# Justin900429/autonomous_driving_with_diffusion_model

Measured on AMD Instinct MI355X. Metric: denoising-steps/sec, higher is better.
Workload: dtype f32

## Files before the change

### autonomous_driving_with_diffusion_model_amd/csrc/conv2d_hs.hip

```cpp
#include <type_traits>
#include <stdlib.h>

#include "adx_common.h"
#include "conv2d_internal.h"
#include "conv2d_hs_common.h"

namespace adx {

template <bool AFFINE = true>
__device__ __forceinline__ void cells_store32(float (&v)[16], const float* sc, const float* sh, int cl0, const float (*res8)[8],
                                              bool relu, __amdgpu_buffer_rsrc_t yrsrc, uint32_t vcell, uint32_t so, uint32_t cplane,
                                              float& amax) {
  float lm = 0.f;
#pragma unroll
  for (int i = 0; i < 2; ++i)
#pragma unroll
    for (int j = 0; j < 4; ++j) {
      const auto sw = __builtin_amdgcn_permlane32_swap(f2u(v[8 * i + j]), f2u(v[8 * i + 4 + j]), false, false);
      v[8 * i + j] = u2f(sw[0]);
      v[8 * i + 4 + j] = u2f(sw[1]);
    }
#pragma unroll
  for (int i = 0; i < 2; ++i) {
    float o[8];
// ... 755 lines not shown
      const u32x4* wa0 = wl + (i & 1) * WST + wa_lane;
      load_w(s + 2 < nstages ? s + 2 : nstages - 1, i & 1);
      if ((i + 1) % 3 < PIT) load_p(s + 4 < nstages ? (s + 4) / 3 : nchunks - 1, (i + 1) % 3, i & 1);
      __builtin_amdgcn_sched_barrier(0);
#pragma unroll
      for (int kw = 0; kw < K; ++kw) {
        f16x8 A[2][2], B[2][2];
#pragma unroll
        for (int pl = 0; pl < 2; ++pl) {
#pragma unroll
          for (int m = 0; m < 2; ++m) A[pl][m] = __builtin_bit_cast(f16x8, wa0[(kw * 2 + pl) * 128 + m * 32]);
#pragma unroll
          for (int r = 0; r < 2; ++r) B[pl][r] = __builtin_bit_cast(f16x8, pb0[pl * PLANE + (r + kh) * PW + kw]);
        }
#pragma unroll
        for (int r = 0; r < 2; ++r)
#pragma unroll
          for (int m = 0; m < 2; ++m) {
            accm[r][m] = hs_mfma(A[0][m], B[0][r], accm[r][m]);
            accl[r][m] = hs_mfma(A[0][m], B[1][r], accl[r][m]);
            accl[r][m] = hs_mfma(A[1][m], B[0][r], accl[r][m]);
          }
        if (kw == 0) {
          store_w((i + 1) & 1, (i + 1) & 1);
          if (i % 3 < PIT) store_p((i + 1) & 1, i % 3, ((i + 3) / 3) & 1);
        }
      }
      __syncthreads();
    }
  }

  HS_TRACE(3);
  const int ox = VROW ? xl : ox0 + ecol;
  const uint32_t plane_ob = (uint32_t)(a.OH * a.OW) * (uint32_t)sizeof(float);
  const size_t img = (size_t)n * a.Cout * a.OH * a.OW;
  const int img_bytes = (int)(uint32_t)((VROW ? (uint32_t)a.N : 1u) * (uint32_t)a.Cout * plane_ob);
  const uint32_t img_off = VROW ? (uint32_t)nl * (uint32_t)a.Cout * plane_ob : 0u;
  float* const ybase = a.ksplit > 1 ? a.part + (size_t)kpart * a.part_stride : a.y;
  const __amdgpu_buffer_rsrc_t yrsrc = __builtin_amdgcn_make_buffer_rsrc(ybase + img, 0, img_bytes, 0x00020000);
  const __amdgpu_buffer_rsrc_t rrsrc = __builtin_amdgcn_make_buffer_rsrc(
      const_cast<float*>(a.res != nullptr ? a.res + img : a.y), 0, a.res != nullptr ? img_bytes : 0, 0x00020000);
  const float* sst = ss + slab * 64;
  const uint32_t cbase_o = (uint32_t)cout0 * plane_ob;
  const uint32_t cplane = (uint32_t)(a.OH * a.OW) * 16u;
  const uint32_t cell0 = (uint32_t)(cout0 >> 3) * 2u * cplane;
  bool inside[2];
  uint32_t pix[2];
#pragma unroll
  for (int rr = 0; rr < 2; ++rr) {
    const int oy = oy0 + rowpair * 2 + rr;
    inside[rr] = lane_valid && oy < a.OH && ox < a.OW;
    pix[rr] = (uint32_t)(oy * a.OW + ox);
  }
  float amax = 0.f;
  if constexpr (YCELLS) {
    const uint32_t khoff = (uint32_t)khalf * 2u * cplane;
    uint32_t vcell[2], vres[2];
#pragma unroll
    for (int rr = 0; rr < 2; ++rr) {
      vcell[rr] = inside[rr] ? img_off + pix[rr] * 16u + khoff : kOutside;
      vres[rr] = !inside[rr] ? kOutside : a.res_cells ? vcell[rr] : img_off + pix[rr] * 4u + (uint32_t)(8 * khalf) * plane_ob;
    }
    uint32_t rraw[2][2][2][8];
#pragma unroll
    for (int rr = 0; rr < 2; ++rr)
#pragma unroll
      for (int half = 0; half < 2; ++half)
#pragma unroll
        for (int i = 0; i < 2; ++i) {
          if (a.res_cells) {
            const uint32_t so = cell0 + (uint32_t)(half * 4 + 2 * i) * 2u * cplane;
            const u32x4 h4 = __builtin_amdgcn_raw_buffer_load_b128(rrsrc, vres[rr], so, 0);
            const u32x4 l4 = __builtin_amdgcn_raw_buffer_load_b128(rrsrc, vres[rr], so + cplane, 0);
#pragma unroll
            for (int j = 0; j < 4; ++j) { rraw[rr][half][i][j] = h4[j]; rraw[rr][half][i][4 + j] = l4[j]; }
          } else {
#pragma unroll
            for (int j = 0; j < 8; ++j)
              rraw[rr][half][i][j] = __builtin_amdgcn_raw_buffer_load_b32(rrsrc, vres[rr], cbase_o + (uint32_t)(half * 32 + 16 * i + j) * plane_ob, 0);
          }
        }
#ifdef ADX_HS_TRACE
    asm volatile("s_waitcnt vmcnt(0)" ::: "memory");
    HS_TRACE(6);
#endif
#pragma unroll
    for (int rr = 0; rr < 2; ++rr)
#pragma unroll
      for (int half = 0; half < 2; ++half) {
        float v[16];
#pragma unroll
        for (int r = 0; r < 16; ++r) v[r] = accm[rr][half][r] + accl[rr][half][r] * (1.f / kLoScale);
        float res8[2][8];
#pragma unroll
        for (int i = 0; i < 2; ++i) {
          if (a.res_cells) {
            half4(rraw[rr][half][i][0], rraw[rr][half][i][1], rraw[rr][half][i][4], rraw[rr][half][i][5], res8[i]);
            half4(rraw[rr][half][i][2], rraw[rr][half][i][3], rraw[rr][half][i][6], rraw[rr][half][i][7], res8[i] + 4);
          } else {
#pragma unroll
            for (int j = 0; j < 8; ++j) res8[i][j] = u2f(rraw[rr][half][i][j]);
          }
        }
        cells_store32(v, sst, sst + 64 * CT, half * 32 + 8 * khalf, res8, a.relu != 0, yrsrc, vcell[rr],
                      cell0 + (uint32_t)(half * 4) * 2u * cplane, cplane, amax);
      }
  } else {
  uint32_t voff[2];
#pragma unroll
  for (int rr = 0; rr < 2; ++rr) voff[rr] = inside[rr] ? img_off + pix[rr] * 4u + (uint32_t)(4 * khalf) * plane_ob : kOutside;
  float rv[2][2][16];
  if constexpr (STATS != 2) {
#pragma unroll
  for (int rr = 0; rr < 2; ++rr)
#pragma unroll
    for (int half = 0; half < 2; ++half)
#pragma unroll
      for (int r = 0; r < 16; ++r) {
        const int cu = half * 32 + (r & 3) + 8 * (r >> 2);
        rv[rr][half][r] = __builtin_bit_cast(float, __builtin_amdgcn_raw_buffer_load_b32(rrsrc, voff[rr], cbase_o + cu * plane_ob, 0));
      }
  }
#ifdef ADX_HS_TRACE
  asm volatile("s_waitcnt vmcnt(0)" ::: "memory");
  HS_TRACE(6);
#endif
  if constexpr (STATS != 0) {
    float* red = reinterpret_cast<float*>(smem_raw);
    const bool val0 = voff[0] != kOutside, val1 = voff[1] != kOutside;
    auto park = [&](int half, int r, float sm, float sq) {
      sm += hs_dpp<0xB1>(sm);  sq += hs_dpp<0xB1>(sq);
      sm += hs_dpp<0x4E>(sm);  sq += hs_dpp<0x4E>(sq);
      sm += hs_dpp<0x141>(sm); sq += hs_dpp<0x141>(sq);
      sm += hs_dpp<0x140>(sm); sq += hs_dpp<0x140>(sq);
      if ((lane & 15) == 0) {
        float* d = red + (((wave * 4 + (lane >> 4)) * 32) + half * 16 + r) * 2;
        d[0] = sm;
        d[1] = sq;
      }
    };
    if constexpr (STATS == 1) {
#pragma unroll
      for (int half = 0; half < 2; ++half)
#pragma unroll
        for (int r = 0; r < 16; ++r) {
          const float v0 = val0 ? (accm[0][half][r] + accl[0][half][r] * (1.f / kLoScale)) * xs_inv : 0.f;
          const float v1 = val1 ? (accm[1][half][r] + accl[1][half][r] * (1.f / kLoScale)) * xs_inv : 0.f;
          park(half, r, v0 + v1, v0 * v0 + v1 * v1);
        }
    } else {
#pragma unroll
      for (int rr = 0; rr < 2; ++rr)
#pragma unroll
        for (int half = 0; half < 2; ++half)
#pragma unroll
          for (int r = 0; r < 16; ++r) accm[rr][half][r] = (accm[rr][half][r] + accl[rr][half][r] * (1.f / kLoScale)) * xs_inv;
      const __amdgpu_buffer_rsrc_t wrsrc = __builtin_amdgcn_make_buffer_rsrc(const_cast<float*>(a.bs_raw + img), 0, img_bytes, 0x00020000);
      const bool mask_bits = a.bs_mask == 1 && a.bs_bits != nullptr;
      const bool mask_out = a.bs_mask == 1 && !mask_bits;
      const __amdgpu_buffer_rsrc_t orsrc = __builtin_amdgcn_make_buffer_rsrc(
          const_cast<float*>(mask_out ? a.bs_out + img : a.y), 0, mask_out ? img_bytes : 0, 0x00020000);
      const uint32_t bplane = (uint32_t)(a.OH * a.OW);
      const __amdgpu_buffer_rsrc_t brsrc = __builtin_amdgcn_make_buffer_rsrc(
          const_cast<uint8_t*>(mask_bits ? a.bs_bits + (size_t)n * (a.Cout >> 3) * bplane : reinterpret_cast<const uint8_t*>(a.y)), 0,
          mask_bits ? (int)((VROW ? (uint32_t)a.N : 1u) * (uint32_t)(a.Cout >> 3) * bplane) : 0, 0x00020000);
      uint32_t boff[2];
#pragma unroll
      for (int rr = 0; rr < 2; ++rr)
        boff[rr] = inside[rr] ? (VROW ? (uint32_t)nl * (uint32_t)(a.Cout >> 3) * bplane : 0u) + pix[rr] : kOutside;
      const bool res_masked = a.res_bits != nullptr;
      const __amdgpu_buffer_rsrc_t qrsrc = __builtin_amdgcn_make_buffer_rsrc(
          const_cast<uint8_t*>(res_masked ? a.res_bits + (size_t)n * (a.Cout >> 3) * bplane : reinterpret_cast<const uint8_t*>(a.y)), 0,
          res_masked ? (int)((VROW ? (uint32_t)a.N : 1u) * (uint32_t)(a.Cout >> 3) * bplane) : 0, 0x00020000);
      const float* bsw = bsl + slab * 64;
      const uint32_t use_bit = mask_bits ? 1u : 0u, use_out = mask_out ? 1u : 0u, use_raw = 1u - use_bit - use_out;
      const uint32_t v0u = val0 ? 1u : 0u, v1u = val1 ? 1u : 0u;
      float dmx = 0.f;
#pragma unroll
      for (int half = 0; half < 2; ++half) {
        float rs_[2][16], rw_[2][16], ro_[2][16];
#pragma unroll
        for (int rr = 0; rr < 2; ++rr)
#pragma unroll
          for (int r = 0; r < 16; ++r) {
            const uint32_t so = cbase_o + (uint32_t)(half * 32 + (r & 3) + 8 * (r >> 2)) * plane_ob;
            rs_[rr][r] = __builtin_bit_cast(float, __builtin_amdgcn_raw_buffer_load_b32(rrsrc, voff[rr], so, 0));
            rw_[rr][r] = __builtin_bit_cast(float, __builtin_amdgcn_raw_buffer_load_b32(wrsrc, voff[rr], so, 0));
            ro_[rr][r] = 0.f;
          }
        if (mask_out) {
#pragma unroll
          for (int rr = 0; rr < 2; ++rr)
#pragma unroll
            for (int r = 0; r < 16; ++r) {
              const uint32_t so = cbase_o + (uint32_t)(half * 32 + (r & 3) + 8 * (r >> 2)) * plane_ob;
              ro_[rr][r] = __builtin_bit_cast(float, __builtin_amdgcn_raw_buffer_load_b32(orsrc, voff[rr], so, 0));
            }
        }
        if (res_masked) {
#pragma unroll
          for (int rr = 0; rr < 2; ++rr)
#pragma unroll
            for (int q = 0; q < 4; ++q) {
              const uint32_t m = (uint32_t)__builtin_amdgcn_raw_buffer_load_b8(qrsrc, boff[rr], ((uint32_t)(cout0 >> 3) + (uint32_t)(half * 4 + q)) * bplane, 0)
                                 >> (4 * khalf);
#pragma unroll
              for (int i = 0; i < 4; ++i)
                if (!((m >> i) & 1u)) rs_[rr][4 * q + i] = 0.f;
            }
        }
        uint32_t mb[2][4] = {{0u, 0u, 0u, 0u}, {0u, 0u, 0u, 0u}};
        if (mask_bits) {
#pragma unroll
          for (int rr = 0; rr < 2; ++rr)
#pragma unroll
            for (int q = 0; q < 4; ++q)
              mb[rr][q] = (uint32_t)__builtin_amdgcn_raw_buffer_load_b8(brsrc, boff[rr], ((uint32_t)(cout0 >> 3) + (uint32_t)(half * 4 + q)) * bplane, 0)
                          >> (4 * khalf);
        }
#pragma unroll
        for (int r = 0; r < 16; ++r) {
          const int cu = half * 32 + (r & 3) + 8 * (r >> 2);
          const int cl = cu + 4 * khalf;
          const float mu = bsw[cl], rsd = bsw[64 * CT + cl], msc = bsw[2 * 64 * CT + cl], msh = bsw[3 * 64 * CT + cl];
          float p[2], q[2];
#pragma unroll
          for (int rr = 0; rr < 2; ++rr) {
            const float y = accm[rr][half][r] + rs_[rr][r];
            __builtin_amdgcn_raw_buffer_store_b32(__builtin_bit_cast(uint32_t, y), yrsrc, voff[rr], cbase_o + cu * plane_ob, 0);
            const uint32_t on_bit = (mb[rr][r >> 2] >> (r & 3)) & 1u, on_out = ro_[rr][r] > 0.f ? 1u : 0u;
            const uint32_t on_raw = __builtin_fmaf(rw_[rr][r], msc, msh) > 0.f ? 1u : 0u;
            const bool keep = ((rr == 0 ? v0u : v1u) & ((on_bit & use_bit) | (on_out & use_out) | (on_raw & use_raw))) != 0u;
            p[rr] = keep ? y : 0.f;
            q[rr] = p[rr] * ((rw_[rr][r] - mu) * rsd);
            dmx = __builtin_fmaxf(dmx, __builtin_fabsf(p[rr]));
          }
          park(half, r, p[0] + p[1], q[0] + q[1]);
        }
      }
#pragma unroll
      for (int off = 32; off > 0; off >>= 1) dmx = __builtin_fmaxf(dmx, __shfl_xor(dmx, off, 64));
      if (lane == 0) red[4096 + wave] = dmx;
    }
    __syncthreads();
    if (STATS == 2 && tid >= 2 * 64 * CT && tid < 2 * 64 * CT + CT) {
      const int sl = tid - 2 * 64 * CT;
      constexpr int WPS = (NT / 64) / CT;
      float t = 0.f;
#pragma unroll
      for (int w = 0; w < WPS; ++w) t = __builtin_fmaxf(t, red[4096 + (MODE == 2 ? sl * WPS + w : w)]);
      const int p = (n * a.tiles_y + ty) * a.tiles_x + tx;
      a.stats_part[(size_t)a.Cout * 2 * a.stats_p + (size_t)(ct * CT + sl) * a.stats_p + p] = t;
    }
    if (tid < 2 * 64 * CT) {
      const int which = tid & 1, chs = tid >> 1, sl = chs >> 6, ch = chs & 63;
      const int c5 = ch & 31, kh2 = (c5 >> 2) & 1, r = (c5 & 3) + 4 * (c5 >> 3), idx32 = (ch >> 5) * 16 + r;
      constexpr int WPS = (NT / 64) / CT;
      float t = 0.f;
#pragma unroll
      for (int w = 0; w < WPS; ++w)
#pragma unroll
        for (int j = 0; j < 2; ++j) t += red[((((MODE == 2 ? sl * WPS + w : w) * 4 + kh2 * 2 + j) * 32) + idx32) * 2 + which];
      const int p = (n * a.tiles_y + ty) * a.tiles_x + tx;
      a.stats_part[((size_t)((ct * CT + sl) * kHsCout + ch) * 2 + which) * a.stats_p + p] = t;
    }
  }
  auto finish = [&](auto relu) {
#pragma unroll
    for (int rr = 0; rr < 2; ++rr) {
      float lm = 0.f;
#pragma unroll
      for (int half = 0; half < 2; ++half)
#pragma unroll
        for (int r = 0; r < 16; ++r) {
          const int cu = half * 32 + (r & 3) + 8 * (r >> 2);
          const int cl = cu + 4 * khalf;
          float v = (accm[rr][half][r] + accl[rr][half][r] * (1.f / kLoScale)) * xs_inv;
          v = v * sst[cl] + sst[64 * CT + cl];
          v += rv[rr][half][r];
          if (decltype(relu)::value) v = __builtin_fmaxf(v, 0.f);
          lm = fp16_amax(lm, v);
          __builtin_amdgcn_raw_buffer_store_b32(__builtin_bit_cast(uint32_t, v), yrsrc, voff[rr], cbase_o + cu * plane_ob, 0);
        }
      amax = fp16_amax(amax, inside[rr] ? lm : 0.f);
    }
  };
  if constexpr (STATS != 2) {
    if (a.relu) finish(std::true_type{}); else finish(std::false_type{});
  }
  }
  range_flag(a.status, out_of_fp16(amax));
  HS_TRACE(4);
#ifdef ADX_HS_TRACE
  __builtin_amdgcn_s_waitcnt(0);
  asm volatile("s_waitcnt vmcnt(0)" ::: "memory");
  HS_TRACE(5);
#endif
}

constexpr int kStemSteps = 11;
constexpr int kStemPP = 72;
constexpr int kStemPH = 21;

struct StemFrags { f16x8 A[2][2], B[2]; };
__device__ __forceinline__ void stem_tile(const u32x4* wa0, const uint32_t* pb0, int khalf, f32x16 (&accm)[2], f32x16 (&accl)[2]) {
  constexpr int CP = kStemPH * kStemPP, PLANEH = 3 * CP;
#pragma unroll
  for (int m = 0; m < 2; ++m)
#pragma unroll
    for (int i = 0; i < 16; ++i) { accm[m][i] = 0.f; accl[m][i] = 0.f; }
  auto fetch = [&](StemFrags& f, int step) {
    const int c0 = 2 * step, c1 = 2 * step + 1 > 20 ? 20 : 2 * step + 1;
    const int off0 = ((c0 / 7) * CP + (c0 % 7) * kStemPP) / 2, off1 = ((c1 / 7) * CP + (c1 % 7) * kStemPP) / 2;
    const uint32_t* pb = pb0 + (khalf ? off1 : off0);
#pragma unroll
    for (int pl = 0; pl < 2; ++pl) {
#pragma unroll
      for (int m = 0; m < 2; ++m) f.A[pl][m] = __builtin_bit_cast(f16x8, wa0[(step * 2 + pl) * 128 + m * 32]);
      const uint32_t* q = pb + pl * (PLANEH / 2);
      u32x4 v;
      v[0] = q[0]; v[1] = q[1]; v[2] = q[2]; v[3] = q[3];
      f.B[pl] = __builtin_bit_cast(f16x8, v);
    }
  };
  StemFrags fr[2];
  fetch(fr[0], 0);
#pragma unroll
  for (int step = 0; step < kStemSteps; ++step) {
    if (step + 1 < kStemSteps) fetch(fr[(step + 1) & 1], step + 1);
    __builtin_amdgcn_sched_barrier(0);
    const StemFrags& f = fr[step & 1];
#pragma unroll
    for (int m = 0; m < 2; ++m) {
      accm[m] = hs_mfma(f.A[0][m], f.B[0], accm[m]);
      accl[m] = hs_mfma(f.A[0][m], f.B[1], accl[m]);
      accl[m] = hs_mfma(f.A[1][m], f.B[0], accl[m]);
    }
    __builtin_amdgcn_sched_barrier(0);
  }
}

constexpr int kStemStageItems = 3 * kStemPH / 7;
template <bool U8>
struct StemStager {
  float pv[kStemStageItems][2];
  float amax = 0.f;
  __device__ __forceinline__ void load(const Conv2dArgs& a, __amdgpu_buffer_rsrc_t xrsrc, int r0, int ix, int iy0) {
    constexpr uint32_t kOutside = 0xC0000000u;
    const bool act = r0 < 7;
    const bool ok0 = act && ix >= 0 && ix < a.W, ok1 = act && ix + 1 >= 0 && ix + 1 < a.W;
    const size_t hw = (size_t)a.H * a.W;
#pragma unroll
    for (int k = 0; k < kStemStageItems; ++k) {
      const int rc = r0 + 7 * k;
      const int c = (rc >= kStemPH) + (rc >= 2 * kStemPH), iy = iy0 + rc - kStemPH * c;
      const bool rok = iy >= 0 && iy < a.H;
      const bool v0 = rok && ok0, v1 = rok && ok1;
      if (U8) {
#pragma clang fp contract(off)
        const uint32_t brow = (uint32_t)(iy * a.W) * 3u + (uint32_t)c;
        const uint32_t b0 = __builtin_amdgcn_raw_buffer_load_b8(xrsrc, v0 ? brow + (uint32_t)ix * 3u : kOutside, 0, 0);
        const uint32_t b1 = __builtin_amdgcn_raw_buffer_load_b8(xrsrc, v1 ? brow + (uint32_t)(ix + 1) * 3u : kOutside, 0, 0);
        const float mean = c == 0 ? a.u8_mean[0] : (c == 1 ? a.u8_mean[1] : a.u8_mean[2]);
        const float stdv = c == 0 ? a.u8_std[0] : (c == 1 ? a.u8_std[1] : a.u8_std[2]);
        pv[k][0] = v0 ? ((float)b0 / 255.0f - mean) / stdv : 0.f;
        pv[k][1] = v1 ? ((float)b1 / 255.0f - mean) / stdv : 0.f;
      } else {
        const uint32_t grow = (uint32_t)(c * (int)hw + iy * a.W) * 4u;
        pv[k][0] = __builtin_bit_cast(float, __builtin_amdgcn_raw_buffer_load_b32(xrsrc, v0 ? grow + (uint32_t)ix * 4u : kOutside, 0, 0));
        pv[k][1] = __builtin_bit_cast(float, __builtin_amdgcn_raw_buffer_load_b32(xrsrc, v1 ? grow + (uint32_t)(ix + 1) * 4u : kOutside, 0, 0));
      }
    }
  }
  __device__ __forceinline__ void store(uint32_t* pd, int r0, int pp) {
    constexpr int PLANEH = 3 * kStemPH * kStemPP;
    if (r0 >= 7) return;
#pragma unroll
    for (int k = 0; k < kStemStageItems; ++k) {
      f16x2 h, l;
#pragma unroll
      for (int j = 0; j < 2; ++j) {
        const _Float16 hj = (_Float16)pv[k][j];
        amax = fp16_amax(amax, pv[k][j]);
        h[j] = hj;
        l[j] = (_Float16)((pv[k][j] - (float)hj) * kLoScale);
      }
      const int dw = ((r0 + 7 * k) * kStemPP) / 2 + pp;
      pd[dw] = __builtin_bit_cast(uint32_t, h);
      pd[PLANEH / 2 + dw] = __builtin_bit_cast(uint32_t, l);
    }
  }
};

__global__ void __launch_bounds__(256, 2) conv2d_hs_stem_kernel(const Conv2dArgs a) {
  constexpr int CP = kStemPH * kStemPP;
  constexpr int PLANEH = 3 * CP;
  extern __shared__ __attribute__((aligned(16))) unsigned char smem_raw[];
  u32x4* wl = reinterpret_cast<u32x4*>(smem_raw);
  uint32_t* patch = reinterpret_cast<uint32_t*>(wl + kStemSteps * 256);
  float* ss = reinterpret_cast<float*>(patch + 2 * PLANEH);
  const int tid = threadIdx.x, lane = tid & 63;
  const int wave = __builtin_amdgcn_readfirstlane(tid >> 6);
  const int l31 = lane & 31, khalf = lane >> 5;
  int bid = blockIdx.x, seg = 0;
  if (a.stem_nseg > 1) { seg = bid % a.stem_nseg; bid /= a.stem_nseg; }
  const int n = bid / a.tiles_y, ty = bid - n * a.tiles_y;
  const int tx_begin = a.stem_nseg > 1 ? seg * a.stem_seg_tiles : 0;
  const int tx_end = a.stem_nseg > 1 ? min(a.tiles_x, tx_begin + a.stem_seg_tiles) : a.tiles_x;
  const int oy0 = ty * 8, iy0 = oy0 * 2 - 3;
  const size_t hw = (size_t)a.H * a.W;
  const __amdgpu_buffer_rsrc_t xrsrc =
      __builtin_amdgcn_make_buffer_rsrc(const_cast<float*>(a.x + (size_t)n * 3 * hw), 0, (int)(3 * hw * sizeof(float)), 0x00020000);

  {
    const u32x4* wsrc = reinterpret_cast<const u32x4*>(a.w);
#pragma unroll
    for (int k = 0; k < kStemSteps; ++k) wl[tid + 256 * k] = wsrc[tid + 256 * k];
  }
  if (tid < 2 * kHsCout) {
    const int c = tid & (kHsCout - 1);
    ss[tid] = a.scale == nullptr ? (tid < kHsCout ? 1.f : 0.f) : (tid < kHsCout ? a.scale[c] : a.shift[c]);
  }
  const int r0 = tid / 35, pp = tid - r0 * 35;
  StemStager<false> sg;
  const u32x4* wa0 = wl + khalf * 64 + l31;
  const size_t img = (size_t)n * a.Cout * a.OH * a.OW;
  const uint32_t plane_ob = (uint32_t)(a.OH * a.OW) * (uint32_t)sizeof(float);
  const __amdgpu_buffer_rsrc_t yrsrc = __builtin_amdgcn_make_buffer_rsrc(a.y + img, 0, (int)(a.Cout * plane_ob), 0x00020000);
  constexpr uint32_t kOutside = 0xC0000000u;

  sg.load(a, xrsrc, r0, tx_begin * 64 - 3 + 2 * pp, iy0);
  sg.store(patch + (tx_begin & 1) * PLANEH, r0, pp);
  __syncthreads();
  for (int tx = tx_begin; tx < tx_end; ++tx) {
    if (tx + 1 < tx_end) sg.load(a, xrsrc, r0, (tx + 1) * 64 - 3 + 2 * pp, iy0);
    const int ox = tx * kTileW + l31;
    const uint32_t* pb0 = patch + (tx & 1) * PLANEH + wave * 4 * (kStemPP / 2) + l31;
    f32x16 accm[2][2], accl[2][2];
#pragma unroll
    for (int r = 0; r < 2; ++r)
#pragma unroll
      for (int m = 0; m < 2; ++m)
#pragma unroll
        for (int i = 0; i < 16; ++i) { accm[r][m][i] = 0.f; accl[r][m][i] = 0.f; }
#pragma unroll 1
    for (int step = 0; step < kStemSteps; ++step) {
      const int c0 = 2 * step, c1 = 2 * step + 1 > 20 ? 20 : 2 * step + 1;
      const int off0 = ((c0 / 7) * CP + (c0 % 7) * kStemPP) / 2, off1 = ((c1 / 7) * CP + (c1 % 7) * kStemPP) / 2;
      const uint32_t* pb = pb0 + (khalf ? off1 : off0);
      f16x8 A[2][2], B[2][2];
#pragma unroll
      for (int pl = 0; pl < 2; ++pl) {
#pragma unroll
        for (int m = 0; m < 2; ++m) A[pl][m] = __builtin_bit_cast(f16x8, wa0[(step * 2 + pl) * 128 + m * 32]);
#pragma unroll
        for (int r = 0; r < 2; ++r) {
          const uint32_t* q = pb + pl * (PLANEH / 2) + r * 2 * (kStemPP / 2);
          u32x4 v;
          v[0] = q[0]; v[1] = q[1]; v[2] = q[2]; v[3] = q[3];
          B[pl][r] = __builtin_bit_cast(f16x8, v);
        }
      }
#pragma unroll
      for (int r = 0; r < 2; ++r)
#pragma unroll
        for (int m = 0; m < 2; ++m) {
          accm[r][m] = hs_mfma(A[0][m], B[0][r], accm[r][m]);
          accl[r][m] = hs_mfma(A[0][m], B[1][r], accl[r][m]);
          accl[r][m] = hs_mfma(A[1][m], B[0][r], accl[r][m]);
        }
    }
#pragma unroll
    for (int rr = 0; rr < 2; ++rr) {
      const int oy = oy0 + wave * 2 + rr;
      const uint32_t voff = (oy < a.OH && ox < a.OW) ? (uint32_t)(oy * a.OW + ox) * 4u + (uint32_t)(4 * khalf) * plane_ob : kOutside;
#pragma unroll
      for (int half = 0; half < 2; ++half)
#pragma unroll
        for (int r = 0; r < 16; ++r) {
          const int cu = half * 32 + (r & 3) + 8 * (r >> 2);
          const int cl = cu + 4 * khalf;
          float v = accm[rr][half][r] + accl[rr][half][r] * (1.f / kLoScale);
          v = v * ss[cl] + ss[kHsCout + cl];
          if (a.relu) v = v > 0.f ? v : 0.f;
          __builtin_amdgcn_raw_buffer_store_b32(__builtin_bit_cast(uint32_t, v), yrsrc, voff, cu * plane_ob, 0);
        }
    }
    if (tx + 1 < tx_end) sg.store(patch + ((tx + 1) & 1) * PLANEH, r0, pp);
    __syncthreads();
  }
}

constexpr int kStemPoolCols = 15;
template <bool U8>
__global__ void __launch_bounds__(256, 2) conv2d_hs_stem_pool_kernel(const Conv2dArgs a) {
  constexpr int PLANEH = 3 * kStemPH * kStemPP;
  extern __shared__ __attribute__((aligned(16))) unsigned char smem_raw[];
  u32x4* wl = reinterpret_cast<u32x4*>(smem_raw);
  uint32_t* patch = reinterpret_cast<uint32_t*>(wl + kStemSteps * 256);
  float* ss = reinterpret_cast<float*>(patch + PLANEH);
  float* xch = ss + 2 * kHsCout;
  const int tid = threadIdx.x, lane = tid & 63;
  const int wave = __builtin_amdgcn_readfirstlane(tid >> 6);
  const int l31 = lane & 31, khalf = lane >> 5;
  int bid = blockIdx.x, seg = 0;
  if (a.stem_nseg > 1) { seg = bid % a.stem_nseg; bid /= a.stem_nseg; }
  const int n = bid / a.tiles_x, tx = bid - n * a.tiles_x;
  const int b_own = a.stem_nseg > 1 ? seg * a.stem_seg_tiles : 0;
  const int b_end = a.stem_nseg > 1 ? min(a.tiles_y, b_own + a.stem_seg_tiles) : a.tiles_y;
  const int b_begin = b_own > 0 ? b_own - 1 : 0;
  const int sx0 = tx * 2 * kStemPoolCols - 1;
  const size_t hw = (size_t)a.H * a.W;
  const __amdgpu_buffer_rsrc_t xrsrc =
      U8 ? __builtin_amdgcn_make_buffer_rsrc(const_cast<uint8_t*>(a.x_u8 + (size_t)n * 3 * hw), 0, (int)(3 * hw), 0x00020000)
         : __builtin_amdgcn_make_buffer_rsrc(const_cast<float*>(a.x + (size_t)n * 3 * hw), 0, (int)(3 * hw * sizeof(float)), 0x00020000);

  {
    const u32x4* wsrc = reinterpret_cast<const u32x4*>(a.w);
#pragma unroll
    for (int k = 0; k < kStemSteps; ++k) wl[tid + 256 * k] = wsrc[tid + 256 * k];
  }
  if (tid < 2 * kHsCout) {
    const int c = tid & (kHsCout - 1);
    ss[tid] = a.scale == nullptr ? (tid < kHsCout ? 1.f : 0.f) : (tid < kHsCout ? a.scale[c] : a.shift[c]);
  }
  const int r0 = tid / 35, pp = tid - r0 * 35;
  const int ix = 2 * sx0 - 3 + 2 * pp;
  StemStager<U8> sg;
  const u32x4* wa0 = wl + khalf * 64 + l31;
  const uint32_t* pb0 = patch + wave * 4 * (kStemPP / 2) + l31;

  const int PHo = (a.OH - 1) / 2 + 1, PWo = (a.OW - 1) / 2 + 1;
  const size_t img = (size_t)n * a.Cout * PHo * PWo;
  const uint32_t plane_ob = (uint32_t)(PHo * PWo) * (uint32_t)sizeof(float);
  const __amdgpu_buffer_rsrc_t yrsrc = __builtin_amdgcn_make_buffer_rsrc(a.y + img, 0, (int)(a.Cout * plane_ob), 0x00020000);
  constexpr uint32_t kOutside = 0xC0000000u;
  const int sx = sx0 + l31, pq = tx * kStemPoolCols + (l31 >> 1);
  const bool col_in = sx >= 0 && sx < a.OW;
  const bool col_st = (l31 & 1) != 0 && l31 < 2 * kStemPoolCols && pq < PWo;
  float* xl = xch + khalf * 16 + (l31 >> 1);

#ifdef ADX_HS_TRACE
  long long tr_c = 0, tr_e = 0, tr_s = 0, tr_t = 0;
  unsigned long long* tr = g_hs_trace + (size_t)(8192 + (blockIdx.x & 8191)) * 8;
  if (threadIdx.x == 0) tr[0] = __builtin_readcyclecounter();
#endif
  sg.load(a, xrsrc, r0, ix, b_begin * 16 - 3);
  sg.store(patch, r0, pp);
  __syncthreads();
#ifdef ADX_HS_TRACE
  if (threadIdx.x == 0) tr[1] = __builtin_readcyclecounter();
#endif
  float vm[32];
#pragma unroll
  for (int j = 0; j < 32; ++j) vm[j] = -INFINITY;
  float oamax = 0.f;
  for (int b = b_begin; b < b_end; ++b) {
#ifdef ADX_HS_TRACE
    tr_t = (long long)__builtin_readcyclecounter();
#endif
    const bool pre = b < b_own;
    if (b + 1 < b_end) sg.load(a, xrsrc, r0, ix, (b + 1) * 16 - 3);
    auto stem_row = [&](auto odd) {
      constexpr int rr = decltype(odd)::value ? 1 : 0;
      f32x16 accm[2], accl[2];
      stem_tile(wa0, pb0 + rr * 2 * (kStemPP / 2), khalf, accm, accl);
      const int oy = b * 8 + 2 * wave + rr;
      const float hi = oy < a.OH && col_in ? INFINITY : -INFINITY;
      float hv[32];
#pragma unroll
      for (int half = 0; half < 2; ++half)
#pragma unroll
        for (int r = 0; r < 16; ++r) {
          const int cl = half * 32 + (r & 3) + 8 * (r >> 2) + 4 * khalf;
          float t = (accm[half][r] + accl[half][r] * (1.f / kLoScale)) * ss[cl] + ss[kHsCout + cl];
          t = __builtin_fminf(__builtin_fmaxf(t, 0.f), hi);
          const int ti = __builtin_bit_cast(int, t);
          const float left = __builtin_bit_cast(float, __builtin_amdgcn_mov_dpp(ti, 0x138 , 0xf, 0xf, true));
          const float right = __builtin_bit_cast(float, __builtin_amdgcn_mov_dpp(ti, 0x130 , 0xf, 0xf, true));
          const int j = half * 16 + r;
          hv[j] = __builtin_fmaxf(__builtin_fmaxf(left, t), right);
          vm[j] = __builtin_fmaxf(vm[j], hv[j]);
        }
      if constexpr (rr == 1) {
        if (l31 & 1) {
#pragma unroll
          for (int j = 0; j < 32; ++j) xl[wave * 1024 + 32 * j] = hv[j];
        }
      }
    };
    if (!pre) stem_row(std::false_type{});
    stem_row(std::true_type{});
#ifdef ADX_HS_TRACE
    { const long long t = (long long)__builtin_readcyclecounter(); tr_c += t - tr_t; tr_t = t; }
#endif
    __syncthreads();
    {
      const float* src = xl + ((wave + 3) & 3) * 1024;
      float up[32];
#pragma unroll
      for (int j = 0; j < 32; ++j) up[j] = src[32 * j];
      if (wave != 0) {
#pragma unroll
        for (int j = 0; j < 32; ++j) vm[j] = __builtin_fmaxf(up[j], vm[j]);
      }
      const int pr = b * 4 + wave;
      if (!pre && pr < PHo) {
        const bool st = col_st;
        if (!a.y_cells) {
          const uint32_t voff = st ? (uint32_t)(pr * PWo + pq) * 4u + (uint32_t)(4 * khalf) * plane_ob : kOutside;
#pragma unroll
          for (int half = 0; half < 2; ++half)
#pragma unroll
            for (int r = 0; r < 16; ++r) {
              const int cu = half * 32 + (r & 3) + 8 * (r >> 2);
              oamax = fp16_amax(oamax, st ? vm[half * 16 + r] : 0.f);
              __builtin_amdgcn_raw_buffer_store_b32(__builtin_bit_cast(uint32_t, vm[half * 16 + r]), yrsrc, voff, cu * plane_ob, 0);
            }
        } else {
          const uint32_t cplane = (uint32_t)(PHo * PWo) * 16u;
          const uint32_t vcell = st ? (uint32_t)(pr * PWo + pq) * 16u + (uint32_t)khalf * 2u * cplane : kOutside;
#pragma unroll
          for (int half = 0; half < 2; ++half) {
            float mm[16];
#pragma unroll
            for (int r = 0; r < 16; ++r) mm[r] = st ? vm[half * 16 + r] : 0.f;
            cells_store32<false>(mm, nullptr, nullptr, 0, nullptr, false, yrsrc, vcell, (uint32_t)(half * 4) * 2u * cplane, cplane, oamax);
          }
        }
      }
#pragma unroll
      for (int j = 0; j < 32; ++j) vm[j] = wave == 0 ? up[j] : -INFINITY;
    }
#ifdef ADX_HS_TRACE
    { const long long t = (long long)__builtin_readcyclecounter(); tr_e += t - tr_t; tr_t = t; }
#endif
    if (b + 1 < b_end) sg.store(patch, r0, pp);
    __syncthreads();
#ifdef ADX_HS_TRACE
    { const long long t = (long long)__builtin_readcyclecounter(); tr_s += t - tr_t; tr_t = t; }
#endif
  }
#ifdef ADX_HS_TRACE
  if (threadIdx.x == 0) {
    tr[2] = (unsigned long long)tr_c;
    tr[3] = (unsigned long long)tr_e;
    tr[4] = (unsigned long long)tr_s;
    tr[5] = __builtin_readcyclecounter();
  }
#endif
  range_flag(a.status, out_of_fp16(fp16_amax(sg.amax, oamax)));
}

__global__ void conv2d_hs_stem_pack_kernel(const float* __restrict__ w, _Float16* __restrict__ p, uint32_t* status) {
  const int idx = blockIdx.x * 256 + threadIdx.x;
  if (idx >= kStemSteps * 2 * 64 * 8) return;
  const int j = idx & 7, ml = (idx >> 3) & 63, h = (idx >> 9) & 1, step = idx >> 10;
  const int combo = 2 * step + h;
  float v = 0.f;
  if (combo < 21 && j < 7) v = w[((size_t)ml * 3 + combo / 7) * 49 + (combo % 7) * 7 + j];
  const _Float16 hi = (_Float16)v;
  const _Float16 lo = (_Float16)((v - (float)hi) * kLoScale);
  const size_t cell = ((size_t)(step * 2 + 0) * 2 + h) * 64 + ml;
  p[cell * 8 + j] = hi;
  p[(cell + 128) * 8 + j] = lo;
  range_flag(status, out_of_fp16(v));
}

static bool hs_is_stem(const ConvSpec& L) { return L.k == 7 && L.stride == 2 && L.pad == 3 && L.cin == 3 && L.cout == 64; }

__global__ void conv2d_hs_pack_kernel(const float* __restrict__ w, _Float16* __restrict__ p, int M, int Kc, int Kreal,
                                      int taps, int dgrad, size_t total, uint32_t* status) {
  const size_t idx = (size_t)blockIdx.x * 256 + threadIdx.x;
  if (idx >= total) return;
  const int j = idx & 7;
  const int ml = (idx >> 3) & 63;
  const int h = (idx >> 9) & 1;
  size_t rest = idx >> 10;
  const int tap = rest % taps; rest /= taps;
  const int nchunks = Kc / kHsCC;
  const int chunk = rest % nchunks;
  const int ct = rest / nchunks;
  const int m = ct * 64 + ml, kc = chunk * kHsCC + h * 8 + j;
  float v = 0.f;
  if (kc < Kreal) v = dgrad ? w[((size_t)kc * M + m) * taps + (taps - 1 - tap)] : w[((size_t)m * Kreal + kc) * taps + tap];
  const _Float16 hi = (_Float16)v;
  const _Float16 lo = (_Float16)((v - (float)hi) * kLoScale);
  const size_t cell = ((((size_t)(ct * nchunks + chunk) * taps + tap) * 2 + 0) * 2 + h) * 64 + ml;
  p[cell * 8 + j] = hi;
  p[(cell + 128) * 8 + j] = lo;
  range_flag(status, out_of_fp16(v));
}

constexpr int kHsPackJobs = 48;
struct HsPackTable {
  const float* w[kHsPackJobs];
  _Float16* p[kHsPackJobs];
  int M[kHsPackJobs], Kc[kHsPackJobs], Kreal[kHsPackJobs], taps[kHsPackJobs], dgrad[kHsPackJobs];
  unsigned first[kHsPackJobs + 1];
  int n;
};
__global__ void __launch_bounds__(256) conv2d_hs_pack_many_kernel(const HsPackTable t) {
  int j = 0, jend = t.n;
  while (jend - j > 1) {
    const int mid = (j + jend) >> 1;
    if (blockIdx.x >= t.first[mid]) j = mid; else jend = mid;
  }
  const int M = t.M[j], Kc = t.Kc[j], Kreal = t.Kreal[j], taps = t.taps[j], dgrad = t.dgrad[j];
  const float* __restrict__ w = t.w[j];
  _Float16* __restrict__ p = t.p[j];
  const size_t total = (size_t)M * Kc * taps;
  const size_t idx = (size_t)(blockIdx.x - t.first[j]) * 256 + threadIdx.x;
  if (idx >= total) return;
  const int e = idx & 7;
  const int ml = (idx >> 3) & 63;
  const int h = (idx >> 9) & 1;
  size_t rest = idx >> 10;
  const int tap = rest % taps; rest /= taps;
  const int nchunks = Kc / kHsCC;
  const int chunk = rest % nchunks;
  const int ct = rest / nchunks;
  const int m = ct * 64 + ml, kc = chunk * kHsCC + h * 8 + e;
  float v = 0.f;
  if (kc < Kreal) v = dgrad ? w[((size_t)kc * M + m) * taps + (taps - 1 - tap)] : w[((size_t)m * Kreal + kc) * taps + tap];
  const _Float16 hi = (_Float16)v;
  const _Float16 lo = (_Float16)((v - (float)hi) * kLoScale);
  const size_t cell = ((((size_t)(ct * nchunks + chunk) * taps + tap) * 2 + 0) * 2 + h) * 64 + ml;
  p[cell * 8 + e] = hi;
  p[(cell + 128) * 8 + e] = lo;
}

int conv2d_hs_pack_many(const HsPackJob* jobs, int n, hipStream_t s) {
  for (int j0 = 0; j0 < n; j0 += kHsPackJobs) {
    HsPackTable t;
    t.n = std::min(kHsPackJobs, n - j0);
    unsigned blocks = 0;
    for (int j = 0; j < t.n; ++j) {
      const HsPackJob& q = jobs[j0 + j];
      ADX_REQUIRE(q.w != nullptr && q.packed != nullptr && q.cin_pad % kHsCC == 0 && q.cout % kHsCout == 0,
                  "conv2d_hs_pack_many: job %d is not a split-fp16 weight image", j0 + j);
      t.w[j] = q.w; t.p[j] = (_Float16*)q.packed;
      t.M[j] = q.cout; t.Kc[j] = q.cin_pad; t.Kreal[j] = q.cin; t.taps[j] = q.taps; t.dgrad[j] = q.dgrad;
      t.first[j] = blocks;
      blocks += (unsigned)(((size_t)q.cout * q.cin_pad * q.taps + 255) / 256);
    }
    t.first[t.n] = blocks;
    conv2d_hs_pack_many_kernel<<<dim3(blocks), dim3(256), 0, s>>>(t);
    ADX_LAUNCH_CHECK();
  }
  return ADX_OK;
}

static bool hs_eligible(const ConvSpec& L, const DebugSwitches& sw) {
  if (sw.conv_exact) return false;
  if (hs_is_stem(L) && !L.dgrad) return true;
  if (L.cin % kHsCC != 0 || L.cin_pad != L.cin || L.cout % kHsCout != 0) return false;
  return L.k == 3 && (L.stride == 1 || L.stride == 2);
}
bool conv2d_hs_eligible(const ConvSpec& L, const DebugSwitches& sw) { return hs_eligible(L, sw); }

size_t conv2d_packed_floats(const ConvSpec& L) {
  const size_t direct = (size_t)L.k * L.k * L.cin_pad * L.cout;
  return direct;
}

bool conv2d_hs_pack_batchable(const ConvSpec& c, int dgrad) { return conv2d_hs_eligible(c) && !(hs_is_stem(c) && !dgrad); }

int conv2d_hs_pack(const ConvSpec& c, const float* w, void* packed, int dgrad, hipStream_t s) {
  if (hs_is_stem(c) && !dgrad) {
    conv2d_hs_stem_pack_kernel<<<dim3(ceil_div(kStemSteps * 2 * 64 * 8, 256)), dim3(256), 0, s>>>(w, (_Float16*)packed, conv2d_status());
    ADX_LAUNCH_CHECK();
    return ADX_OK;
  }
  const size_t total = (size_t)c.cout * c.cin_pad * c.k * c.k;
  conv2d_hs_pack_kernel<<<dim3((unsigned)((total + 255) / 256)), dim3(256), 0, s>>>(
      w, (_Float16*)packed, c.cout, c.cin_pad, c.cin, c.k * c.k, dgrad, total, conv2d_status());
  ADX_LAUNCH_CHECK();
  return ADX_OK;
}

template <int STRIDE, int K, int ROWS, int PBUF, bool DS, bool XCELLS = false, bool YCELLS = false>
static int hs_launch_t(Conv2dArgs a, hipStream_t s) {
  constexpr int TH = 4 * ROWS;
  constexpr int PH = (TH - 1) * STRIDE + K, PW = (kTileW - 1) * STRIDE + K;
  constexpr size_t lds = (size_t)PBUF * 64 * PH * PW + (size_t)2 * K * 256 * 16 + (DS ? 256 * 16 : 0) +
                         (DS ? 4 : 2) * kHsCout * sizeof(float) + 16;
  static_assert(lds <= 80 * 1024, "two workgroups per CU need <= 80 KB each");
  static std::atomic<uint64_t> attr{0};
  if (DeviceOnce once{attr}; once) {
    ADX_CHECK_HIP(hipFuncSetAttribute(reinterpret_cast<const void*>(&conv2d_hs_kernel<STRIDE, K, ROWS, PBUF, DS, XCELLS, YCELLS>),
                                      hipFuncAttributeMaxDynamicSharedMemorySize, (int)lds));
    once.commit();
  }
  a.tiles_x = ceil_div(a.OW, kTileW); a.tiles_y = ceil_div(a.OH, TH); a.cout_tiles = a.Cout / kHsCout;
  const size_t grid = (size_t)a.cout_tiles * a.tiles_x * a.tiles_y * a.N;
  ADX_REQUIRE(grid < (1u << 31), "conv2d_hs: grid too large");
  ADX_REQUIRE((size_t)a.Cout * a.OH * a.OW * sizeof(float) < 0x7FFFFFFFu, "conv2d_hs: one image of the output exceeds the 32-bit byte offsets");
  conv2d_hs_kernel<STRIDE, K, ROWS, PBUF, DS, XCELLS, YCELLS><<<dim3((unsigned)grid), dim3(256), lds, s>>>(a);
  ADX_LAUNCH_CHECK();
  return ADX_OK;
}

static int hs_stem_launch(Conv2dArgs a, hipStream_t s) {
  constexpr size_t lds = (size_t)kStemSteps * 4096 + (size_t)2 * 4 * 3 * kStemPH * kStemPP + 2 * kHsCout * sizeof(float);
  static_assert(lds <= 80 * 1024, "two workgroups per CU need <= 80 KB each");
  static std::atomic<uint64_t> attr{0};
  if (DeviceOnce once{attr}; once) {
    ADX_CHECK_HIP(hipFuncSetAttribute(reinterpret_cast<const void*>(&conv2d_hs_stem_kernel), hipFuncAttributeMaxDynamicSharedMemorySize,
                                      (int)lds));
    once.commit();
  }
  a.tiles_x = ceil_div(a.OW, kTileW); a.cout_tiles = 1;
  a.tiles_y = ceil_div(a.OH, 8);
  const int bands = a.tiles_y * a.N;
  a.stem_seg_tiles = 0; a.stem_nseg = 1;
  if (bands < 128 && a.tiles_x > 1) {
    const int want = std::min(a.tiles_x, std::max(1, 256 / bands));
    a.stem_seg_tiles = ceil_div(a.tiles_x, want);
    a.stem_nseg = ceil_div(a.tiles_x, a.stem_seg_tiles);
    if (a.stem_nseg <= 1) { a.stem_seg_tiles = 0; a.stem_nseg = 1; }
  }
  conv2d_hs_stem_kernel<<<dim3((unsigned)(bands * a.stem_nseg)), dim3(256), lds, s>>>(a);
  ADX_LAUNCH_CHECK();
  return ADX_OK;
}

template <bool U8>
static int hs_stem_pool_launch(Conv2dArgs a, hipStream_t s) {
  constexpr size_t lds = (size_t)kStemSteps * 4096 + (size_t)4 * 3 * kStemPH * kStemPP + 2 * kHsCout * sizeof(float) +
                         (size_t)4 * 1024 * sizeof(float);
  static_assert(lds <= 80 * 1024, "two workgroups per CU need <= 80 KB each");
  static std::atomic<uint64_t> attr{0};
  if (DeviceOnce once{attr}; once) {
    ADX_CHECK_HIP(hipFuncSetAttribute(reinterpret_cast<const void*>(&conv2d_hs_stem_pool_kernel<U8>),
                                      hipFuncAttributeMaxDynamicSharedMemorySize, (int)lds));
    once.commit();
  }
  a.tiles_x = ceil_div((a.OW - 1) / 2 + 1, kStemPoolCols); a.cout_tiles = 1;
  a.tiles_y = ceil_div((a.OH - 1) / 2 + 1, 4);
  const int strips = a.tiles_x * a.N;
  a.stem_seg_tiles = 0; a.stem_nseg = 1;
  if (strips < 256 && a.tiles_y > 1) {
    const int want = std::min(a.tiles_y, std::max(1, 512 / strips));
    a.stem_seg_tiles = ceil_div(a.tiles_y, want);
    a.stem_nseg = ceil_div(a.tiles_y, a.stem_seg_tiles);
    if (a.stem_nseg <= 1) { a.stem_seg_tiles = 0; a.stem_nseg = 1; }
  }
  conv2d_hs_stem_pool_kernel<U8><<<dim3((unsigned)(strips * a.stem_nseg)), dim3(256), lds, s>>>(a);
  ADX_LAUNCH_CHECK();
  return ADX_OK;
}

int conv2d_hs_stem_pool(const ConvSpec& L, const float* x, const float* w, const float* scale, const float* shift,
                        float* pooled, int N, int H, int W, hipStream_t s, const uint8_t* frames_u8, const float* mean,
                        const float* stdv, int y_cells) {
  ADX_REQUIRE((x || frames_u8) && w && scale && shift && pooled, "conv2d_hs_stem_pool: null pointer");
  ADX_REQUIRE((size_t)3 * H * W * sizeof(float) < 0xC0000000u, "conv2d_hs_stem_pool: image too large for 32-bit offsets");
  Conv2dArgs a{};
  a.x = x; a.w = w; a.scale = scale; a.shift = shift; a.y = pooled;
  if (frames_u8 != nullptr) {
    ADX_REQUIRE(mean && stdv, "conv2d_hs_stem_pool: uint8 frames need mean / std");
    a.x_u8 = frames_u8;
    for (int c = 0; c < 3; ++c) { a.u8_mean[c] = mean[c]; a.u8_std[c] = stdv[c]; }
  }
  a.N = N; a.Cin = 3; a.H = H; a.W = W; a.Cout = 64;
  a.OH = conv_out_dim(H, 7, 2, 3); a.OW = conv_out_dim(W, 7, 2, 3);
  a.KH = 7; a.KW = 7; a.stride = 2; a.pad = 3; a.relu = 1;
  a.cin_pad = L.cin_pad; a.cc = L.cc;
  a.y_cells = y_cells;
  a.status = conv2d_status();
  return frames_u8 != nullptr ? hs_stem_pool_launch<true>(a, s) : hs_stem_pool_launch<false>(a, s);
}

int conv2d_hs_launch_block_s2(const ConvSpec& c1, const ConvSpec& ds, const float* x, const float* w1, const float* scale1,
                              const float* shift1, float* y1, const float* wd, const float* scaled, const float* shiftd,
                              float* yd, int N, int H, int W, hipStream_t s, int x_cells, int y_cells, int relu, bool force_32) {
  ADX_REQUIRE(x && w1 && y1 && wd && yd && (scale1 != nullptr) == (shift1 != nullptr) && (scaled != nullptr) == (shiftd != nullptr),
              "conv2d_hs block launch: null pointer");
  Conv2dArgs a{};
  a.x = x; a.w = w1; a.scale = scale1; a.shift = shift1; a.res = nullptr; a.y = y1; a.x_amax = nullptr; a.x_amax_n = 0;
  a.w_ds = wd; a.scale_ds = scaled; a.shift_ds = shiftd; a.y_ds = yd;
  a.N = N; a.Cin = c1.cin; a.H = H; a.W = W; a.Cout = c1.cout;
  a.OH = conv_out_dim(H, 3, 2, 1); a.OW = conv_out_dim(W, 3, 2, 1);
  a.KH = 3; a.KW = 3; a.stride = 2; a.pad = 1; a.relu = relu;
  a.cin_pad = c1.cin_pad; a.cc = c1.cc;
  a.x_cells = x_cells;
  a.y_cells = y_cells;
  a.status = conv2d_status();
  HsS2Query q;
  q.N = N; q.H = H; q.W = W; q.x_cells = x_cells != 0; q.y_cells = y_cells != 0;
  if (q.x_cells && q.y_cells && !force_32) {
    const int rc = launch_cus(&q.cus);
    if (rc != ADX_OK) return rc;
    const HsS2Plan plan = conv2d_hs_s2_plan(c1, ds, q);
    if (plan.q) return conv2d_hs3x3q_s2_launch(plan, a, s);
  }
  return conv2d_hs_launch(c1, a, s);
}

HsS2Plan conv2d_hs_s2_plan(const ConvSpec& c1, const ConvSpec& ds, const HsS2Query& q, const DebugSwitches& sw) {
  HsS2Plan p;
  const bool shape = hs_eligible(c1, sw) && c1.k == 3 && c1.stride == 2 && c1.pad == 1 && ds.k == 1 && ds.stride == 2 && ds.pad == 0 &&
                     ds.cin == c1.cin && ds.cout == c1.cout && c1.cin_pad % 64 == 0 && c1.cout % 128 == 0;
  if (!shape || !q.x_cells || !q.y_cells || !sw.hs_s2q || !sw.hs_dma || sw.hs_mode >= 0 || q.N < 1 || q.H < 1 || q.W < 1) return p;
  const int N = q.N, OH = conv_out_dim(q.H, 3, 2, 1), OW = conv_out_dim(q.W, 3, 2, 1);
  if ((size_t)N * c1.cin * q.H * q.W * sizeof(float) >= 0xC0000000u || (size_t)N * c1.cout * OH * OW * sizeof(float) >= 0xC0000000u ||
      (long)N * (OW + 1) >= (1L << 21))
    return p;
  p.q = true;
  p.vw = N > 1 ? OW + 1 : OW;
  p.tiles_x = (int)(((long)N * p.vw - (N > 1 ? 1 : 0) + kTileW - 1) / kTileW);
  p.tiles_y = ceil_div(OH, kQTH);
  p.cout_tiles = c1.cout / 128;
  p.q_slots = hs3x3q_slots(p.cout_tiles * p.tiles_x * p.tiles_y, q.cus, sw.hs_persist);
  p.grid = (size_t)8 * p.q_slots;
  p.threads = kQNT;
  p.lds = kQLdsS2;
  return p;
}

__global__ void __launch_bounds__(256) conv2d_split_reduce_kernel(const float* __restrict__ part, size_t part_stride, int nparts,
                                                                  const float* __restrict__ scale, const float* __restrict__ shift,
                                                                  const float* __restrict__ res, float* __restrict__ y,
                                                                  int cout, int plane4, size_t total4, int relu, uint32_t* status) {
  const size_t i = (size_t)blockIdx.x * 256 + threadIdx.x;
  if (i >= total4) return;
  const int c = (int)((i / plane4) % cout);
  f32x4 v = reinterpret_cast<const f32x4*>(part)[i];
  for (int p0 = 1; p0 < nparts; p0 += 8) {
    f32x4 t[8];
#pragma unroll
    for (int j = 0; j < 8; ++j) t[j] = reinterpret_cast<const f32x4*>(part + (size_t)(p0 + j < nparts ? p0 + j : 0) * part_stride)[i];
#pragma unroll
    for (int j = 0; j < 8; ++j)
      if (p0 + j < nparts) v += t[j];
  }
  const float sc = scale != nullptr ? scale[c] : 1.f, sh = shift != nullptr ? shift[c] : 0.f;
  v = v * sc + sh;
  if (res != nullptr) v += reinterpret_cast<const f32x4*>(res)[i];
  if (relu) {
#pragma unroll
    for (int k = 0; k < 4; ++k) v[k] = __builtin_fmaxf(v[k], 0.f);
  }
  reinterpret_cast<f32x4*>(y)[i] = v;
  float amax = 0.f;
#pragma unroll
  for (int k = 0; k < 4; ++k) amax = fp16_amax(amax, v[k]);
  range_flag(status, out_of_fp16(amax));
}

static constexpr size_t hs3x3_lds(int mode, int stats, bool pair = false) {
  const int th = mode == 1 ? 16 : 8, ct = mode == 2 ? 2 : 1;
  const size_t patch = pair ?(size_t)2 * 2 * kHsPairKHalf * 16 : (size_t)2 * 64 * (th + 2) * 34;
  return patch + (size_t)2 * (pair ? 2 : 3 * ct) * 256 * 16 + (2 * 64 * ct + 8) * sizeof(float) + 48 +
// ... 217 lines not shown
```

Baseline: 178.9.

## Fuse stem conv rows into one MFMA tile sharing weight fragments

Adds stem_tile2, which computes both output rows of a block in one pass, so A-fragment weight loads are shared across the two rows and LDS loads are interleaved between MFMA groups. It also precomputes LDS lane bases with explicit LDS address-space pointers, pins the u8 mean/std in scalar registers, and carries the pooled row across iterations through LDS instead of registers. The status flag now uses a wave ballot so only one lane issues the atomic. This raises register pressure from the doubled accumulators, which may reduce occupancy.

```diff
diff --git a/autonomous_driving_with_diffusion_model_amd/csrc/conv2d_hs.hip b/autonomous_driving_with_diffusion_model_amd/csrc/conv2d_hs.hip
--- a/autonomous_driving_with_diffusion_model_amd/csrc/conv2d_hs.hip
+++ b/autonomous_driving_with_diffusion_model_amd/csrc/conv2d_hs.hip
@@ -1081,22 +1081,39 @@
 constexpr int kStemPP = 72;
 constexpr int kStemPH = 21;
 
+typedef __attribute__((address_space(3))) const uint32_t lds_u32;
+struct StemPatchBase {
+  static constexpr int CP = kStemPH * kStemPP, PLANEH = 3 * CP;
+  static constexpr int DROW = kStemPP / 2, DCH = (CP - 6 * kStemPP) / 2;
+  const uint32_t *p0, *prow, *pch;
+  __device__ __forceinline__ StemPatchBase(const uint32_t* pb0, int khalf) {
+    asm volatile("" : "+v"(khalf));
+    p0 = pb0; prow = pb0 + khalf * DROW; pch = pb0 + khalf * DCH;
+  }
+  __device__ __forceinline__ lds_u32* at(int step, int pl) const {
+    const int c0 = 2 * step, c1 = 2 * step + 1 > 20 ? 20 : 2 * step + 1;
+    const int off0 = ((c0 / 7) * CP + (c0 % 7) * kStemPP) / 2, off1 = ((c1 / 7) * CP + (c1 % 7) * kStemPP) / 2;
+    const int d = off1 - off0;
+    const uint32_t* const lane_base = d == DROW ? prow : (d == DCH ? pch : p0);
+    uint32_t addr = (uint32_t)(uintptr_t)(lds_u32*)(lane_base + off0 + pl * (PLANEH / 2));
+    asm volatile("" : "+v"(addr));
+    return (lds_u32*)(uintptr_t)addr;
+  }
+};
+
 struct StemFrags { f16x8 A[2][2], B[2]; };
 __device__ __forceinline__ void stem_tile(const u32x4* wa0, const uint32_t* pb0, int khalf, f32x16 (&accm)[2], f32x16 (&accl)[2]) {
-  constexpr int CP = kStemPH * kStemPP, PLANEH = 3 * CP;
 #pragma unroll
   for (int m = 0; m < 2; ++m)
 #pragma unroll
     for (int i = 0; i < 16; ++i) { accm[m][i] = 0.f; accl[m][i] = 0.f; }
+  const StemPatchBase pb(pb0, khalf);
   auto fetch = [&](StemFrags& f, int step) {
-    const int c0 = 2 * step, c1 = 2 * step + 1 > 20 ? 20 : 2 * step + 1;
-    const int off0 = ((c0 / 7) * CP + (c0 % 7) * kStemPP) / 2, off1 = ((c1 / 7) * CP + (c1 % 7) * kStemPP) / 2;
-    const uint32_t* pb = pb0 + (khalf ? off1 : off0);
 #pragma unroll
     for (int pl = 0; pl < 2; ++pl) {
 #pragma unroll
       for (int m = 0; m < 2; ++m) f.A[pl][m] = __builtin_bit_cast(f16x8, wa0[(step * 2 + pl) * 128 + m * 32]);
-      const uint32_t* q = pb + pl * (PLANEH / 2);
+      lds_u32* q = pb.at(step, pl);
       u32x4 v;
       v[0] = q[0]; v[1] = q[1]; v[2] = q[2]; v[3] = q[3];
       f.B[pl] = __builtin_bit_cast(f16x8, v);
@@ -1116,6 +1133,60 @@
       accl[m] = hs_mfma(f.A[1][m], f.B[0], accl[m]);
     }
     __builtin_amdgcn_sched_barrier(0);
+  }
+}
+
+__device__ __forceinline__ void stem_tile2(const u32x4* wa0, const uint32_t* pb0, int khalf, f32x16 (&accm)[2][2], f32x16 (&accl)[2][2]) {
+#pragma unroll
+  for (int r = 0; r < 2; ++r)
+#pragma unroll
+    for (int m = 0; m < 2; ++m)
+#pragma unroll
+      for (int i = 0; i < 16; ++i) { accm[r][m][i] = 0.f; accl[r][m][i] = 0.f; }
+  auto loadA = [&](int step, int pl, int m) { return __builtin_bit_cast(f16x8, wa0[(step * 2 + pl) * 128 + m * 32]); };
+  const StemPatchBase pb(pb0, khalf);
+  auto baseB = [&](int step, int pl) { return pb.at(step, pl); };
+  auto loadB = [&](lds_u32* base, int r) {
+    lds_u32* q = base + r * 2 * (kStemPP / 2);
+    u32x4 v;
+    v[0] = q[0]; v[1] = q[1]; v[2] = q[2]; v[3] = q[3];
+    return __builtin_bit_cast(f16x8, v);
+  };
+  f16x8 A0[2], A1[2], B0[2], B1[2];
+  {
+    lds_u32 *b0 = baseB(0, 0), *b1 = baseB(0, 1);
+#pragma unroll
+    for (int i = 0; i < 2; ++i) { B1[i] = loadB(b1, i); A0[i] = loadA(0, 0, i); }
+#pragma unroll
+    for (int i = 0; i < 2; ++i) { B0[i] = loadB(b0, i); A1[i] = loadA(0, 1, i); }
+  }
+#pragma unroll
+  for (int step = 0; step < kStemSteps; ++step) {
+    const bool more = step + 1 < kStemSteps;
+    __builtin_amdgcn_sched_barrier(0);
+#pragma unroll
+    for (int r = 0; r < 2; ++r)
+#pragma unroll
+      for (int m = 0; m < 2; ++m) accl[r][m] = hs_mfma(A0[m], B1[r], accl[r][m]);
+    __builtin_amdgcn_sched_barrier(0);
+    if (more) { lds_u32* b1 = baseB(step + 1, 1); B1[0] = loadB(b1, 0); B1[1] = loadB(b1, 1); }
+    __builtin_amdgcn_sched_barrier(0);
+#pragma unroll
+    for (int r = 0; r < 2; ++r)
+#pragma unroll
+      for (int m = 0; m < 2; ++m) accm[r][m] = hs_mfma(A0[m], B0[r], accm[r][m]);
+    __builtin_amdgcn_sched_barrier(0);
+    if (more) { A0[0] = loadA(step + 1, 0, 0); A0[1] = loadA(step + 1, 0, 1); }
+    __builtin_amdgcn_sched_barrier(0);
+#pragma unroll
+    for (int r = 0; r < 2; ++r)
+#pragma unroll
+      for (int m = 0; m < 2; ++m) accl[r][m] = hs_mfma(A1[m], B0[r], accl[r][m]);
+    __builtin_amdgcn_sched_barrier(0);
+    if (more) {
+      lds_u32* b0 = baseB(step + 1, 0);
+      B0[0] = loadB(b0, 0); B0[1] = loadB(b0, 1); A1[0] = loadA(step + 1, 1, 0); A1[1] = loadA(step + 1, 1, 1);
+    }
   }
 }
 
@@ -1140,8 +1211,10 @@
         const uint32_t brow = (uint32_t)(iy * a.W) * 3u + (uint32_t)c;
         const uint32_t b0 = __builtin_amdgcn_raw_buffer_load_b8(xrsrc, v0 ? brow + (uint32_t)ix * 3u : kOutside, 0, 0);
         const uint32_t b1 = __builtin_amdgcn_raw_buffer_load_b8(xrsrc, v1 ? brow + (uint32_t)(ix + 1) * 3u : kOutside, 0, 0);
-        const float mean = c == 0 ? a.u8_mean[0] : (c == 1 ? a.u8_mean[1] : a.u8_mean[2]);
-        const float stdv = c == 0 ? a.u8_std[0] : (c == 1 ? a.u8_std[1] : a.u8_std[2]);
+        float m0 = a.u8_mean[0], m1 = a.u8_mean[1], m2 = a.u8_mean[2], s0 = a.u8_std[0], s1 = a.u8_std[1], s2 = a.u8_std[2];
+        asm volatile("" : "+s"(m0), "+s"(m1), "+s"(m2), "+s"(s0), "+s"(s1), "+s"(s2));
+        const float mean = c == 0 ? m0 : (c == 1 ? m1 : m2);
+        const float stdv = c == 0 ? s0 : (c == 1 ? s1 : s2);
         pv[k][0] = v0 ? ((float)b0 / 255.0f - mean) / stdv : 0.f;
         pv[k][1] = v1 ? ((float)b1 / 255.0f - mean) / stdv : 0.f;
       } else {
@@ -1330,20 +1403,27 @@
 #ifdef ADX_HS_TRACE
   if (threadIdx.x == 0) tr[1] = __builtin_readcyclecounter();
 #endif
-  float vm[32];
-#pragma unroll
-  for (int j = 0; j < 32; ++j) vm[j] = -INFINITY;
   float oamax = 0.f;
   for (int b = b_begin; b < b_end; ++b) {
 #ifdef ADX_HS_TRACE
     tr_t = (long long)__builtin_readcyclecounter();
 #endif
     const bool pre = b < b_own;
-    if (b + 1 < b_end) sg.load(a, xrsrc, r0, ix, (b + 1) * 16 - 3);
-    auto stem_row = [&](auto odd) {
+    const bool next = b + 1 < b_end;
+    int r0b = r0;
+    asm volatile("" : "+v"(r0b));
+    float vm[32];
+    auto vm_begin = [&]() {
+      if (wave == 0 && b > b_begin) {
+#pragma unroll
+        for (int j = 0; j < 32; ++j) vm[j] = xl[32 * j];
+      } else {
+#pragma unroll
+        for (int j = 0; j < 32; ++j) vm[j] = -INFINITY;
+      }
+    };
+    auto stem_row = [&](auto odd, const f32x16 (&accm)[2], const f32x16 (&accl)[2]) {
       constexpr int rr = decltype(odd)::value ? 1 : 0;
-      f32x16 accm[2], accl[2];
-      stem_tile(wa0, pb0 + rr * 2 * (kStemPP / 2), khalf, accm, accl);
       const int oy = b * 8 + 2 * wave + rr;
       const float hi = oy < a.OH && col_in ? INFINITY : -INFINITY;
       float hv[32];
@@ -1368,15 +1448,27 @@
         }
       }
     };
-    if (!pre) stem_row(std::false_type{});
-    stem_row(std::true_type{});
+    if (pre) {
+      if (next) sg.load(a, xrsrc, r0b, ix, (b + 1) * 16 - 3);
+      f32x16 accm[2], accl[2];
+      stem_tile(wa0, pb0 + 2 * (kStemPP / 2), khalf, accm, accl);
+      vm_begin();
+      stem_row(std::true_type{}, accm, accl);
+    } else {
+      f32x16 accm[2][2], accl[2][2];
+      stem_tile2(wa0, pb0, khalf, accm, accl);
+      if (next) sg.load(a, xrsrc, r0b, ix, (b + 1) * 16 - 3);
+      vm_begin();
+      stem_row(std::false_type{}, accm[0], accl[0]);
+      stem_row(std::true_type{}, accm[1], accl[1]);
+    }
 #ifdef ADX_HS_TRACE
     { const long long t = (long long)__builtin_readcyclecounter(); tr_c += t - tr_t; tr_t = t; }
 #endif
     __syncthreads();
+    float up[32];
     {
       const float* src = xl + ((wave + 3) & 3) * 1024;
-      float up[32];
 #pragma unroll
       for (int j = 0; j < 32; ++j) up[j] = src[32 * j];
       if (wave != 0) {
@@ -1403,19 +1495,21 @@
           for (int half = 0; half < 2; ++half) {
             float mm[16];
 #pragma unroll
-            for (int r = 0; r < 16; ++r) mm[r] = st ? vm[half * 16 + r] : 0.f;
+            for (int r = 0; r < 16; ++r) mm[r] = vm[half * 16 + r];
             cells_store32<false>(mm, nullptr, nullptr, 0, nullptr, false, yrsrc, vcell, (uint32_t)(half * 4) * 2u * cplane, cplane, oamax);
           }
         }
       }
-#pragma unroll
-      for (int j = 0; j < 32; ++j) vm[j] = wave == 0 ? up[j] : -INFINITY;
     }
 #ifdef ADX_HS_TRACE
     { const long long t = (long long)__builtin_readcyclecounter(); tr_e += t - tr_t; tr_t = t; }
 #endif
     if (b + 1 < b_end) sg.store(patch, r0, pp);
     __syncthreads();
+    if (wave == 0 && next && (l31 & 1)) {
+#pragma unroll
+      for (int j = 0; j < 32; ++j) xl[32 * j] = up[j];
+    }
 #ifdef ADX_HS_TRACE
     { const long long t = (long long)__builtin_readcyclecounter(); tr_s += t - tr_t; tr_t = t; }
 #endif
@@ -1428,7 +1522,11 @@
     tr[5] = __builtin_readcyclecounter();
   }
 #endif
-  range_flag(a.status, out_of_fp16(fp16_amax(sg.amax, oamax)));
+  if (a.status != nullptr) {
+    const unsigned long long m = __ballot(out_of_fp16(fp16_amax(sg.amax, oamax)));
+    const int ln = (int)__builtin_amdgcn_mbcnt_hi(~0u, __builtin_amdgcn_mbcnt_lo(~0u, 0u));
+    if (m != 0ull && ln == __ffsll(m) - 1) atomicOr(a.status, 1u);
+  }
 }
 
 __global__ void conv2d_hs_stem_pack_kernel(const float* __restrict__ w, _Float16* __restrict__ p, uint32_t* status) {
```

Result: no change. 180.0, median of 5 (+0.6%).
